# saiprasadbarke/robustmvd

Hardware: AMD Instinct MI355X
Metric: depth-maps/sec at 768x1152x4srcx256planes; warp+aggregate HBM GB/s vs roofline (higher is better)
Workload: dtype f32; 1 GPU; mvsnet (Path B) forward 768x1152, 4 source views, 256 planes, batch 1 per step (BASELINE.json configs[2]); the regulariser's two layers with 32 input channels (conv0, conv4): every fp32 operand as two range-scaled fp16 terms on fp16 MFMA, fp32 accumulation (at least as close to a float64 convolution as the fp32 matrix instruction over 1e-42..1e30: tests/test_hip_f16.py), the other nine layers and ; parallelism=1 independent replica(s), frames round-robin, no collectives

## Files before the change

robustmvd_amd/csrc/conv3d_split.hip:

```cpp
#include "mvd_common.h"
#include "split_operand.h"

#ifndef SPLIT_KO
#define SPLIT_KO 0
#endif
#ifndef SPLIT_DEPTH
#define SPLIT_DEPTH 4
#endif

namespace mvd {

typedef _Float16 h16x8 __attribute__((ext_vector_type(8)));
typedef float sf32x4 __attribute__((ext_vector_type(4)));
typedef unsigned int su32x4 __attribute__((ext_vector_type(4)));
typedef unsigned int su32x2 __attribute__((ext_vector_type(2)));
typedef _Float16 h16x2 __attribute__((ext_vector_type(2)));

constexpr int S_TH = 4, S_TW = 32, S_ROWS = S_TH + 2;
constexpr float S_LO_FACTOR = 2048.0f;
template <int CIN>
struct SplitGeom {
    static constexpr int CH8 = CIN / 8;
    static constexpr int VB = CIN * 2;
    static constexpr int KWG = CIN == 32 ? 3 : 2;
    static constexpr int NT = 9 * KWG;
    static constexpr int COLS = CIN == 32 ? S_TW + 2 : S_TW + 3;
    static constexpr int HALF_BYTES = S_ROWS * COLS * VB;
    static constexpr int PLANE_BYTES = 2 * HALF_BYTES;
    static constexpr int ITEMS = S_ROWS * COLS * CH8;
    static constexpr int NLOAD = (ITEMS + 255) / 256;
    static constexpr int NF = 4 * KWG * 2;
    static_assert(NF - 8 == 4 * NLOAD, "pass B interleaves 8 epilogue groups and 4 staging groups per item");
};

template <int CIN>
__global__ void pack_conv0_split_kernel(const float* __restrict__ w, const float* __restrict__ wscale, _Float16* __restrict__ packed, int ncb) {
    using G = SplitGeom<CIN>;
    const int e = blockIdx.x * 256 + threadIdx.x;
    if (e >= ncb * G::NT * 64 * 8) return;
    const int j = e & 7, lane = (e >> 3) & 63, t = (e >> 9) % G::NT, cb = (e >> 9) / G::NT;
    const int col = lane & 15, k = 8 * (lane >> 4) + j, cout = cb * 8 + (col & 7);
    int tap, cin;
    if constexpr (CIN == 32) { tap = t; cin = k; }
    else { const int kw = 2 * (t % 2) + k / 16; tap = kw < 3 ? (t / 2) * 3 + kw : -1; cin = k % 16; }
    const float v = tap >= 0 ? w[((size_t)cout * CIN + cin) * 27 + tap] / wscale[cout] : 0.0f;
    _Float16 hi, lo;
    split_weight(v, S_LO_FACTOR, hi, lo);
    packed[e] = col < 8 ? hi : lo;
}

struct SplitParams {
    const float* x;
    const char* wpk;
    const float* scale;
    const float* shift;
    const float* absmax;
    float* y;
    float* yamax;
    int B, D, h, w, relu;
    int cout, ncb;
    int tiles_x, tiles_y, dgroups, td, tiles_per_xcd;
};

__device__ __forceinline__ unsigned pack_h2(_Float16 a, _Float16 b) {
    const h16x2 v = {a, b};
    return __builtin_bit_cast(unsigned, v);
}

template <int CIN, bool YAMAX = false>
__global__ void __launch_bounds__(256, 2) conv0_split_kernel(SplitParams p) {
    using G = SplitGeom<CIN>;
    constexpr int S_COLS = G::COLS, S_HALF_BYTES = G::HALF_BYTES, S_PLANE_BYTES = G::PLANE_BYTES, S_ITEMS = G::ITEMS, S_NLOAD = G::NLOAD;
    constexpr int KWG = G::KWG, NT = G::NT;
    extern __shared__ __attribute__((aligned(16))) char ring[];
    const int tid = threadIdx.x, lane = tid & 63, wv = tid >> 6;
    const int D = p.D, h = p.h, w = p.w;

    const int xcd = blockIdx.x & 7;
    int j = blockIdx.x >> 3;
    const int cb = j % p.ncb; j /= p.ncb;
    const int t_in = j % p.tiles_per_xcd; j /= p.tiles_per_xcd;
    const int dg = j % p.dgroups;
    const int b = j / p.dgroups;
    const int tile = xcd * p.tiles_per_xcd + t_in;
    if (tile >= p.tiles_x * p.tiles_y) return;
    const int ty = tile / p.tiles_x, tx = tile - ty * p.tiles_x;
    const int x0 = tx * S_TW, y0 = ty * S_TH;
    const int dz0 = dg * p.td, dz1 = min(dz0 + p.td, D);

    h16x8 wf[NT];
#pragma unroll
    for (int t = 0; t < NT; ++t) wf[t] = *reinterpret_cast<const h16x8*>(p.wpk + (((size_t)cb * NT + t) * 64 + lane) * 16);

    constexpr unsigned OOB = 0x80000000u;
    unsigned gob[S_NLOAD];
    int loff[S_NLOAD];
#pragma unroll
    for (int k = 0; k < S_NLOAD; ++k) {
        const int e = tid + 256 * k;
        const int vox = e / G::CH8, ch = e % G::CH8;
        const int r = vox / S_COLS, c = vox - r * S_COLS;
        const int gy = y0 - 1 + r, gx = x0 - 1 + c;
        const bool in = e < S_ITEMS && c < S_TW + 2 && gy >= 0 && gy < h && gx >= 0 && gx < w;
        gob[k] = in ? (unsigned)(((gy * w + gx) * CIN + ch * 8) * 4) : OOB;
        if constexpr (CIN == 32) loff[k] = e < S_ITEMS ? (vox * 64 + ((ch ^ ((c >> 1) & 3)) * 16)) : -1;
        else loff[k] = e < S_ITEMS ? e * 16 : -1;
    }
    const size_t plane_f = (size_t)h * w * CIN;
    const float* xb = p.x + (size_t)b * D * plane_f;
    su32x4 pre[S_NLOAD][2];
    auto fetch = [&](int d) {
        const bool din = d >= 0 && d < D && d <= dz1;
        const __amdgpu_buffer_rsrc_t rs = __builtin_amdgcn_make_buffer_rsrc(
            const_cast<float*>(xb + (din ? (size_t)d * plane_f : 0)), 0, din ? (int)(plane_f * 4) : 0, 0x00020000);
#pragma unroll
        for (int k = 0; k < S_NLOAD; ++k) {
            pre[k][0] = __builtin_amdgcn_raw_buffer_load_b128(rs, gob[k], 0, 0);
            pre[k][1] = __builtin_amdgcn_raw_buffer_load_b128(rs, gob[k] + 16u, 0, 0);
        }
    };
    char* const dump = ring + 2 * S_PLANE_BYTES + tid * 16;
    float xs, xs_inv;
    split_xscale(p.absmax, xs, xs_inv);
    auto split2 = [xs](float a0, float a1, unsigned& hi, unsigned& lo) { mvd::split2(xs, a0, a1, hi, lo, S_LO_FACTOR); };
    auto stash = [&](int d) {
        char* slot = ring + (d & 1) * S_PLANE_BYTES;
#pragma unroll
        for (int k = 0; k < S_NLOAD; ++k) {
            su32x4 hv, lv;
#pragma unroll
            for (int q = 0; q < 4; ++q) {
                const sf32x4 v = __builtin_bit_cast(sf32x4, pre[k][q >> 1]);
                unsigned hi, lo;
                split2(v[(q & 1) * 2], v[(q & 1) * 2 + 1], hi, lo);
                hv[q] = hi; lv[q] = lo;
            }
            char* dst = loff[k] >= 0 ? slot + loff[k] : dump;
            *reinterpret_cast<su32x4*>(dst) = hv;
            *reinterpret_cast<su32x4*>(loff[k] >= 0 ? dst + S_HALF_BYTES : dst) = lv;
        }
    };

    const int col = lane & 15;
    float esc_ = p.scale[cb * 8 + (col & 7)], esh_ = p.shift[cb * 8 + (col & 7)];
    float eun_ = reinterpret_cast<const float*>(p.wpk + (size_t)p.ncb * NT * 64 * 16)[cb * 8 + (col & 7)] * xs_inv;
    const float floor_ = p.relu ? 0.f : -__builtin_inff();
    const int xh = wv & 1, rp = wv >> 1;

    int fragk[KWG];
#pragma unroll
    for (int kw = 0; kw < KWG; ++kw) {
        if constexpr (CIN == 32) {
            const int c = 16 * xh + (lane & 15) + kw;
            fragk[kw] = (2 * rp * S_COLS + c) * 64 + (((lane >> 4) ^ ((c >> 1) & 3)) * 16);
        } else {
            const int c = 16 * xh + (lane & 15) + 2 * kw;
            fragk[kw] = (2 * rp * S_COLS + c) * 32 + (lane >> 4) * 16;
        }
    }

    sf32x4 acc[3][2][2];
#pragma unroll
    for (int s = 0; s < 3; ++s)
#pragma unroll
        for (int r = 0; r < 2; ++r) { acc[s][r][0] = sf32x4{0, 0, 0, 0}; acc[s][r][1] = sf32x4{0, 0, 0, 0}; }

    unsigned yoff[2];
#pragma unroll
    for (int row = 0; row < 2; ++row) {
        const int oy = y0 + 2 * rp + row;
        yoff[row] = (col < 8 && oy < h) ? (unsigned)((((size_t)oy * w + x0 + 16 * xh + 4 * (lane >> 4)) * p.cout + cb * 8 + col) * 4) : OOB;
    }
    const int oxb = x0 + 16 * xh + 4 * (lane >> 4);
    const size_t yplane_f = (size_t)h * w * p.cout;
    const unsigned vox_b = (unsigned)p.cout * 4u;

    fetch(dz0 - 1);
    asm volatile("" : "+v"(esc_), "+v"(esh_), "+v"(eun_));
    stash(dz0 - 1);
    fetch(dz0);

    [[maybe_unused]] float amax_ = 0.f;
    for (int z = dz0 - 1; z <= dz1; ++z) {
        if (!(SPLIT_KO & 8)) __syncthreads();
        const char* slot = ring + (z & 1) * S_PLANE_BYTES;
        char* wslot = ring + ((z + 1) & 1) * S_PLANE_BYTES;
        const int din = z + 2, dout = z - 1;
        const bool in_ok = din >= 0 && din < D && din <= dz1, out_ok = dout >= dz0 && dout < dz1;
        const __amdgpu_buffer_rsrc_t rs_in = __builtin_amdgcn_make_buffer_rsrc(
            const_cast<float*>(xb + (in_ok ? (size_t)din * plane_f : 0)), 0, in_ok ? (int)(plane_f * 4) : 0, 0x00020000);
        const __amdgpu_buffer_rsrc_t rs_out = __builtin_amdgcn_make_buffer_rsrc(
            p.y + ((size_t)b * D + (out_ok ? dout : 0)) * yplane_f, 0, out_ok ? (int)(yplane_f * 4) : 0, 0x00020000);
        int ox = oxb;
        asm volatile("" : "+v"(ox));

        constexpr int NF = G::NF, NR = 2 * NF, DEPTH = SPLIT_DEPTH;
        h16x8 fr[DEPTH];
        auto rr_of = [](int ro) { return ro == 0 ? 1 : ro == 1 ? 2 : ro == 2 ? 0 : 3; };
        auto frag = [&](int i) {
            const int g = i % NF, term = g & 1, kw = (g >> 1) % KWG, rr = rr_of(g / (2 * KWG));
            if (SPLIT_KO & 32) return wf[i % NT];
            return *reinterpret_cast<const h16x8*>(slot + term * S_HALF_BYTES + fragk[kw] + rr * S_COLS * G::VB);
        };
#pragma unroll
        for (int i = 0; i < DEPTH; ++i) fr[i] = frag(i);
#pragma unroll
        for (int g = 0; g < NF; ++g) {
            const int term = g & 1, kw = (g >> 1) % KWG, rr = rr_of(g / (2 * KWG));
            const h16x8 f = fr[g % DEPTH];
#pragma unroll
            for (int row = 0; row < 2; ++row) {
                const int kh = rr - row;
                if (kh < 0 || kh > 2) continue;
                if (SPLIT_KO & 16) acc[0][row][term][0] += f[0] * wf[(6 + kh) * KWG + kw][0];
                else acc[0][row][term] = __builtin_amdgcn_mfma_f32_16x16x32_f16(f, wf[(6 + kh) * KWG + kw], acc[0][row][term], 0, 0, 0);
            }
            fr[g % DEPTH] = frag(g + DEPTH);
            __builtin_amdgcn_sched_barrier(0);
        }
        float hl = __shfl_down(acc[0][0][0][0], 8, 16);
        unsigned hq0 = 0, lq0 = 0;
#pragma unroll
        for (int g = 0; g < NF; ++g) {
            const int term = g & 1, kw = (g >> 1) % KWG, rr = rr_of(g / (2 * KWG));
            const h16x8 f = fr[(NF + g) % DEPTH];
#pragma unroll
            for (int row = 0; row < 2; ++row) {
                const int kh = rr - row;
                if (kh < 0 || kh > 2) continue;
#pragma unroll
                for (int s = 1; s < 3; ++s)
                    if (SPLIT_KO & 16) acc[s][row][term][0] += f[0] * wf[((2 - s) * 3 + kh) * KWG + kw][0];
                    else acc[s][row][term] = __builtin_amdgcn_mfma_f32_16x16x32_f16(f, wf[((2 - s) * 3 + kh) * KWG + kw], acc[s][row][term], 0, 0, 0);
            }
            if (NF + g + DEPTH < NR) fr[(NF + g) % DEPTH] = frag(NF + g + DEPTH);
            if (g < 8) {
                const int row = g >> 2, i = g & 3;
                const float cur = hl;
                if (g + 1 < 8) hl = __shfl_down(acc[0][(g + 1) >> 2][0][(g + 1) & 3], 8, 16);
                float r = __builtin_fmaf(cur + acc[0][row][1][i], 1.0f / 2048.0f, acc[0][row][0][i]);
                r = fmaxf(__builtin_fmaf(r * eun_, esc_, esh_), floor_);
                if constexpr (YAMAX)
                    if (out_ok && yoff[row] != OOB && ox + i < w) amax_ = fmaxf(amax_, finite_abs_or_zero(r));
                if (!(SPLIT_KO & 2) || r == 12345.678f)
                    __builtin_amdgcn_raw_buffer_store_b32(__float_as_uint(r), rs_out, ox + i < w ? yoff[row] + vox_b * i : OOB, 0, 0);
            } else if (!(SPLIT_KO & 4)) {
                const int k = (g - 8) >> 2, q = (g - 8) & 3;
                const sf32x4 v = __builtin_bit_cast(sf32x4, pre[k][q >> 1]);
                unsigned hq1, lq1;
                split2(v[(q & 1) * 2], v[(q & 1) * 2 + 1], hq1, lq1);
                if (q & 1) {
                    char* dst = (loff[k] >= 0 ? wslot + loff[k] : dump) + 8 * (q >> 1);
                    *reinterpret_cast<su32x2*>(dst) = su32x2{hq0, hq1};
                    *reinterpret_cast<su32x2*>(loff[k] >= 0 ? dst + S_HALF_BYTES : dst) = su32x2{lq0, lq1};
                } else {
                    hq0 = hq1; lq0 = lq1;
                }
                if (q == 3 && !(SPLIT_KO & 1)) {
                    pre[k][0] = __builtin_amdgcn_raw_buffer_load_b128(rs_in, gob[k], 0, 0);
                    pre[k][1] = __builtin_amdgcn_raw_buffer_load_b128(rs_in, gob[k] + 16u, 0, 0);
                }
            }
            __builtin_amdgcn_sched_barrier(0);
        }
#pragma unroll
        for (int r = 0; r < 2; ++r)
#pragma unroll
            for (int t = 0; t < 2; ++t) {
                acc[0][r][t] = acc[1][r][t];
                acc[1][r][t] = acc[2][r][t];
                acc[2][r][t] = sf32x4{0, 0, 0, 0};
            }
    }
    if constexpr (YAMAX) {
        for (int o = 32; o > 0; o >>= 1) amax_ = fmaxf(amax_, __shfl_xor(amax_, o));
        __syncthreads();
        float* wm = reinterpret_cast<float*>(ring);
        if (lane == 0) wm[wv] = amax_;
        __syncthreads();
        if (tid == 0) {
            amax_ = fmaxf(fmaxf(wm[0], wm[1]), fmaxf(wm[2], wm[3]));
            raise_absmax(p.yamax, amax_);
        }
    }
}

}

static bool split_shape_ok(int Cin, int Cout) { return (Cin == 32 || Cin == 16) && Cout >= 8 && Cout <= 64 && Cout % 8 == 0; }
static size_t split_frag_bytes(int Cin, int Cout) { return (size_t)(Cout / 8) * (Cin == 32 ? 27 : 18) * 64 * 16; }

template <int CIN, bool YAMAX>
static int launch_split_v(const mvd::SplitParams& p, long long nblk, hipStream_t st) {
    const size_t lds = 2 * (size_t)mvd::SplitGeom<CIN>::PLANE_BYTES + 256 * 16;
    (void)hipFuncSetAttribute((const void*)mvd::conv0_split_kernel<CIN, YAMAX>, hipFuncAttributeMaxDynamicSharedMemorySize, (int)lds);
    hipLaunchKernelGGL((mvd::conv0_split_kernel<CIN, YAMAX>), dim3((unsigned)nblk), dim3(256), lds, st, p);
    return mvd::launch_status("conv3d_split");
}
template <int CIN>
static int launch_split(const mvd::SplitParams& p, long long nblk, hipStream_t st) {
    return p.yamax ? launch_split_v<CIN, true>(p, nblk, st) : launch_split_v<CIN, false>(p, nblk, st);
}

extern "C" {

size_t mvd_conv3d_split_packed_weight_bytes(int Cin, int Cout) {
    return split_shape_ok(Cin, Cout) ? split_frag_bytes(Cin, Cout) + (size_t)Cout * sizeof(float) : 0;
}

int mvd_pack_conv3d_weights_split(const float* w, int Cin, int Cout, void* packed, mvd_stream_t stream) {
    MVD_REQUIRE(w && packed, "pack_conv3d_weights_split: NULL argument");
    MVD_REQUIRE(split_shape_ok(Cin, Cout), "pack_conv3d_weights_split: 16 or 32 input channels and 8, 16, ... 64 output channels are built (got %d -> %d)", Cin, Cout);
    const int ncb = Cout / 8;
    float* wscale = reinterpret_cast<float*>(static_cast<char*>(packed) + split_frag_bytes(Cin, Cout));
    mvd::split_wscale_launch(w, wscale, Cin, Cout, 27, false, Cout, Cout, (hipStream_t)stream);
    const unsigned nb = (unsigned)((split_frag_bytes(Cin, Cout) / 2 + 255) / 256);
    if (Cin == 32) hipLaunchKernelGGL(mvd::pack_conv0_split_kernel<32>, dim3(nb), dim3(256), 0, (hipStream_t)stream, w, wscale, (_Float16*)packed, ncb);
    else hipLaunchKernelGGL(mvd::pack_conv0_split_kernel<16>, dim3(nb), dim3(256), 0, (hipStream_t)stream, w, wscale, (_Float16*)packed, ncb);
    return mvd::launch_status("pack_conv3d_weights_split");
}

static int conv3d_split_entry(const float* x, const float* x_absmax, const void* packed_w, const float* scale, const float* shift, float* y,
                              float* y_absmax, int B, int D, int h, int w, int Cin, int Cout, int relu, mvd_stream_t stream);

int mvd_conv3d_bn_relu_f32_split(const float* x, const float* x_absmax, const void* packed_w, const float* scale, const float* shift,
                                 float* y, int B, int D, int h, int w, int Cin, int Cout, int relu, mvd_stream_t stream) {
    return conv3d_split_entry(x, x_absmax, packed_w, scale, shift, y, nullptr, B, D, h, w, Cin, Cout, relu, stream);
}

int mvd_conv3d_bn_relu_absmax_f32_split(const float* x, const float* x_absmax, const void* packed_w, const float* scale, const float* shift,
                                        float* y, float* y_absmax, int B, int D, int h, int w, int Cin, int Cout, int relu,
                                        mvd_stream_t stream) {
    MVD_REQUIRE(y_absmax, "conv3d_split_absmax: NULL argument");
    return conv3d_split_entry(x, x_absmax, packed_w, scale, shift, y, y_absmax, B, D, h, w, Cin, Cout, relu, stream);
}

static int conv3d_split_entry(const float* x, const float* x_absmax, const void* packed_w, const float* scale, const float* shift, float* y,
                              float* y_absmax, int B, int D, int h, int w, int Cin, int Cout, int relu, mvd_stream_t stream) {
    MVD_REQUIRE(x && x_absmax && packed_w && scale && shift && y, "conv3d_split: NULL argument");
    MVD_REQUIRE(split_shape_ok(Cin, Cout), "conv3d_split: 16 or 32 input channels and 8, 16, ... 64 output channels are built (got %d -> %d)", Cin, Cout);
    MVD_REQUIRE(B > 0 && D > 0 && h > 0 && w > 0, "conv3d_split: non-positive dimension");
    MVD_REQUIRE((long long)h * w * Cin * 4 < 0x7fffffffLL && (long long)h * w * Cout * 4 < 0x7fffffffLL,
                "conv3d_split: one plane exceeds the 31-bit byte-offset range");
    mvd::SplitParams p{};
    p.x = x; p.absmax = x_absmax; p.wpk = (const char*)packed_w; p.scale = scale; p.shift = shift; p.y = y; p.yamax = y_absmax;
    if (y_absmax && hipMemsetAsync(y_absmax, 0, sizeof(float), (hipStream_t)stream) != hipSuccess) return mvd::launch_status("conv3d_split: memset");
    p.B = B; p.D = D; p.h = h; p.w = w; p.relu = relu;
    p.cout = Cout; p.ncb = Cout / 8;
    p.tiles_x = (w + mvd::S_TW - 1) / mvd::S_TW;
    p.tiles_y = (h + mvd::S_TH - 1) / mvd::S_TH;
    const long long tiles = (long long)p.tiles_x * p.tiles_y;
    p.tiles_per_xcd = (int)((tiles + 7) / 8);
    int td = 32;
    while (td > 8 && tiles * B * p.ncb * ((D + td - 1) / td) < 2048) td /= 2;
    p.td = td;
    p.dgroups = (D + td - 1) / td;
    const long long nblk = 8LL * p.ncb * p.tiles_per_xcd * p.dgroups * B;
    MVD_REQUIRE(nblk <= 0x7fffffffLL, "conv3d_split: %lld workgroups exceed the grid limit", nblk);
    return Cin == 32 ? launch_split<32>(p, nblk, (hipStream_t)stream) : launch_split<16>(p, nblk, (hipStream_t)stream);
}
}
```

Measured before the change: 358.2 depth-maps/sec.

## Share depth-rolling accumulators across split terms and shift results with DPP rotates

The default path (non-SIX) repacks the weights so each fragment packs hi and lo weight terms for two depth taps in its 16 output columns. The depth-sliding accumulator state then shrinks from six per-term accumulators to five (X, Z, LA, Y, LB), with cross-lane DPP row rotates replacing the old shuffle and register shift between depth planes. This is meant to cut the number of MFMAs per plane and drop the shuffle in the epilogue. The change also adds an env-gated persistent-slot scheduler, a configurable staging point and a legacy switch. These add code complexity and make the weight layout depend on how the kernel is built.

```diff
diff --git a/robustmvd_amd/csrc/conv3d_split.hip b/robustmvd_amd/csrc/conv3d_split.hip
--- a/robustmvd_amd/csrc/conv3d_split.hip
+++ b/robustmvd_amd/csrc/conv3d_split.hip
@@ -1,3 +1,6 @@
+#include <algorithm>
+#include <cstdlib>
+
 #include "mvd_common.h"
 #include "split_operand.h"
 
@@ -6,6 +9,9 @@
 #endif
 #ifndef SPLIT_DEPTH
 #define SPLIT_DEPTH 4
+#endif
+#ifndef SPLIT_STAGE_AT
+#define SPLIT_STAGE_AT 8
 #endif
 
 namespace mvd {
@@ -30,23 +36,34 @@
     static constexpr int ITEMS = S_ROWS * COLS * CH8;
     static constexpr int NLOAD = (ITEMS + 255) / 256;
     static constexpr int NF = 4 * KWG * 2;
-    static_assert(NF - 8 == 4 * NLOAD, "pass B interleaves 8 epilogue groups and 4 staging groups per item");
+    static_assert(NF - 8 == 4 * NLOAD, "a pass has room for 8 epilogue groups and 4 staging groups per item");
 };
 
-template <int CIN>
+template <int CIN, bool SIX>
 __global__ void pack_conv0_split_kernel(const float* __restrict__ w, const float* __restrict__ wscale, _Float16* __restrict__ packed, int ncb) {
     using G = SplitGeom<CIN>;
     const int e = blockIdx.x * 256 + threadIdx.x;
     if (e >= ncb * G::NT * 64 * 8) return;
     const int j = e & 7, lane = (e >> 3) & 63, t = (e >> 9) % G::NT, cb = (e >> 9) / G::NT;
     const int col = lane & 15, k = 8 * (lane >> 4) + j, cout = cb * 8 + (col & 7);
+    int kdkh, g;
+    bool lo_term;
+    if constexpr (SIX) {
+        kdkh = t / G::KWG; g = t % G::KWG; lo_term = col >= 8;
+    } else {
+        const int f = t % 3, kh = (t / 3) / G::KWG;
+        g = (t / 3) % G::KWG;
+        const int kd = f == 1 ? 0 : (col < 8 ? 2 : 1);
+        kdkh = kd * 3 + kh;
+        lo_term = f == 2 || (f == 1 && col >= 8);
+    }
     int tap, cin;
-    if constexpr (CIN == 32) { tap = t; cin = k; }
-    else { const int kw = 2 * (t % 2) + k / 16; tap = kw < 3 ? (t / 2) * 3 + kw : -1; cin = k % 16; }
+    if constexpr (CIN == 32) { tap = kdkh * 3 + g; cin = k; }
+    else { const int kw = 2 * g + k / 16; tap = kw < 3 ? kdkh * 3 + kw : -1; cin = k % 16; }
     const float v = tap >= 0 ? w[((size_t)cout * CIN + cin) * 27 + tap] / wscale[cout] : 0.0f;
     _Float16 hi, lo;
     split_weight(v, S_LO_FACTOR, hi, lo);
-    packed[e] = col < 8 ? hi : lo;
+    packed[e] = lo_term ? lo : hi;
 }
 
 struct SplitParams {
@@ -60,6 +77,8 @@
     int B, D, h, w, relu;
     int cout, ncb;
     int tiles_x, tiles_y, dgroups, td, tiles_per_xcd;
+    int slots;
+    long long total;
 };
 
 __device__ __forceinline__ unsigned pack_h2(_Float16 a, _Float16 b) {
@@ -67,7 +86,12 @@
     return __builtin_bit_cast(unsigned, v);
 }
 
-template <int CIN, bool YAMAX = false>
+template <int BANK_MASK>
+__device__ __forceinline__ float ror8(float keep, float src) {
+    return __builtin_bit_cast(float, __builtin_amdgcn_update_dpp(__builtin_bit_cast(int, keep), __builtin_bit_cast(int, src), 0x128, 0xf, BANK_MASK, false));
+}
+
+template <int CIN, bool YAMAX = false, bool SIX = false>
 __global__ void __launch_bounds__(256, 2) conv0_split_kernel(SplitParams p) {
     using G = SplitGeom<CIN>;
     constexpr int S_COLS = G::COLS, S_HALF_BYTES = G::HALF_BYTES, S_PLANE_BYTES = G::PLANE_BYTES, S_ITEMS = G::ITEMS, S_NLOAD = G::NLOAD;
@@ -77,24 +101,83 @@
     const int D = p.D, h = p.h, w = p.w;
 
     const int xcd = blockIdx.x & 7;
-    int j = blockIdx.x >> 3;
-    const int cb = j % p.ncb; j /= p.ncb;
-    const int t_in = j % p.tiles_per_xcd; j /= p.tiles_per_xcd;
-    const int dg = j % p.dgroups;
-    const int b = j / p.dgroups;
-    const int tile = xcd * p.tiles_per_xcd + t_in;
-    if (tile >= p.tiles_x * p.tiles_y) return;
+    long long lin, lin_end;
+    if (p.slots > 0) {
+        const int q = p.slots >> 3, rem = p.slots & 7;
+        const int rank = (xcd < rem ? xcd * (q + 1) : rem * (q + 1) + (xcd - rem) * q) + (int)(blockIdx.x >> 3);
+        lin = p.total * rank / p.slots;
+        lin_end = p.total * (rank + 1) / p.slots;
+    } else {
+        int j = blockIdx.x >> 3;
+        const int cb = j % p.ncb; j /= p.ncb;
+        const int t_in = j % p.tiles_per_xcd; j /= p.tiles_per_xcd;
+        const int dg = j % p.dgroups;
+        const int b = j / p.dgroups;
+        const int tile = xcd * p.tiles_per_xcd + t_in;
+        if (tile >= p.tiles_x * p.tiles_y) return;
+        lin = (((long long)tile * p.B + b) * p.ncb + cb) * D + dg * p.td;
+        lin_end = lin + min(p.td, D - dg * p.td);
+    }
+
+    constexpr unsigned OOB = 0x80000000u;
+    int loff[S_NLOAD];
+#pragma unroll
+    for (int k = 0; k < S_NLOAD; ++k) {
+        const int e = tid + 256 * k;
+        const int vox = e / G::CH8, ch = e % G::CH8;
+        const int c = vox % S_COLS;
+        if constexpr (CIN == 32) loff[k] = e < S_ITEMS ? (vox * 64 + ((ch ^ ((c >> 1) & 3)) * 16)) : -1;
+        else loff[k] = e < S_ITEMS ? e * 16 : -1;
+    }
+    const size_t plane_f = (size_t)h * w * CIN;
+    char* const dump = ring + 2 * S_PLANE_BYTES + tid * 16;
+    float xs, xs_inv;
+    split_xscale(p.absmax, xs, xs_inv);
+    auto split2 = [xs](float a0, float a1, unsigned& hi, unsigned& lo) { mvd::split2(xs, a0, a1, hi, lo, S_LO_FACTOR); };
+    const int col = lane & 15;
+    const float floor_ = p.relu ? 0.f : -__builtin_inff();
+    const int xh = wv & 1, rp = wv >> 1;
+
+    int fragk[KWG];
+#pragma unroll
+    for (int kw = 0; kw < KWG; ++kw) {
+        if constexpr (CIN == 32) {
+            const int c = 16 * xh + (lane & 15) + kw;
+            fragk[kw] = (2 * rp * S_COLS + c) * 64 + (((lane >> 4) ^ ((c >> 1) & 3)) * 16);
+        } else {
+            const int c = 16 * xh + (lane & 15) + 2 * kw;
+            fragk[kw] = (2 * rp * S_COLS + c) * 32 + (lane >> 4) * 16;
+        }
+    }
+    const size_t yplane_f = (size_t)h * w * p.cout;
+    const unsigned vox_b = (unsigned)p.cout * 4u;
+
+    h16x8 wf[NT];
+    float esc_ = 0.f, esh_ = 0.f, eun_ = 0.f;
+    int cb_resident = -1;
+    [[maybe_unused]] float amax_ = 0.f;
+
+  while (lin < lin_end) {
+    const int dz0 = (int)(lin % D);
+    long long sj = lin / D;
+    const int cb = (int)(sj % p.ncb); sj /= p.ncb;
+    const int b = (int)(sj % p.B);
+    const int tile = (int)(sj / p.B);
+    const int dz1 = (int)min((long long)D, dz0 + (lin_end - lin));
+    lin += dz1 - dz0;
     const int ty = tile / p.tiles_x, tx = tile - ty * p.tiles_x;
     const int x0 = tx * S_TW, y0 = ty * S_TH;
-    const int dz0 = dg * p.td, dz1 = min(dz0 + p.td, D);
-
-    h16x8 wf[NT];
-#pragma unroll
-    for (int t = 0; t < NT; ++t) wf[t] = *reinterpret_cast<const h16x8*>(p.wpk + (((size_t)cb * NT + t) * 64 + lane) * 16);
-
-    constexpr unsigned OOB = 0x80000000u;
+
+    if (cb != cb_resident) {
+        cb_resident = cb;
+#pragma unroll
+        for (int t = 0; t < NT; ++t) wf[t] = *reinterpret_cast<const h16x8*>(p.wpk + (((size_t)cb * NT + t) * 64 + lane) * 16);
+        esc_ = p.scale[cb * 8 + (col & 7)];
+        esh_ = p.shift[cb * 8 + (col & 7)];
+        eun_ = reinterpret_cast<const float*>(p.wpk + (size_t)p.ncb * NT * 64 * 16)[cb * 8 + (col & 7)] * xs_inv;
+    }
+
     unsigned gob[S_NLOAD];
-    int loff[S_NLOAD];
 #pragma unroll
     for (int k = 0; k < S_NLOAD; ++k) {
         const int e = tid + 256 * k;
@@ -103,10 +186,7 @@
         const int gy = y0 - 1 + r, gx = x0 - 1 + c;
         const bool in = e < S_ITEMS && c < S_TW + 2 && gy >= 0 && gy < h && gx >= 0 && gx < w;
         gob[k] = in ? (unsigned)(((gy * w + gx) * CIN + ch * 8) * 4) : OOB;
-        if constexpr (CIN == 32) loff[k] = e < S_ITEMS ? (vox * 64 + ((ch ^ ((c >> 1) & 3)) * 16)) : -1;
-        else loff[k] = e < S_ITEMS ? e * 16 : -1;
-    }
-    const size_t plane_f = (size_t)h * w * CIN;
+    }
     const float* xb = p.x + (size_t)b * D * plane_f;
     su32x4 pre[S_NLOAD][2];
     auto fetch = [&](int d) {
@@ -119,10 +199,6 @@
             pre[k][1] = __builtin_amdgcn_raw_buffer_load_b128(rs, gob[k] + 16u, 0, 0);
         }
     };
-    char* const dump = ring + 2 * S_PLANE_BYTES + tid * 16;
-    float xs, xs_inv;
-    split_xscale(p.absmax, xs, xs_inv);
-    auto split2 = [xs](float a0, float a1, unsigned& hi, unsigned& lo) { mvd::split2(xs, a0, a1, hi, lo, S_LO_FACTOR); };
     auto stash = [&](int d) {
         char* slot = ring + (d & 1) * S_PLANE_BYTES;
 #pragma unroll
@@ -141,29 +217,13 @@
         }
     };
 
-    const int col = lane & 15;
-    float esc_ = p.scale[cb * 8 + (col & 7)], esh_ = p.shift[cb * 8 + (col & 7)];
-    float eun_ = reinterpret_cast<const float*>(p.wpk + (size_t)p.ncb * NT * 64 * 16)[cb * 8 + (col & 7)] * xs_inv;
-    const float floor_ = p.relu ? 0.f : -__builtin_inff();
-    const int xh = wv & 1, rp = wv >> 1;
-
-    int fragk[KWG];
-#pragma unroll
-    for (int kw = 0; kw < KWG; ++kw) {
-        if constexpr (CIN == 32) {
-            const int c = 16 * xh + (lane & 15) + kw;
-            fragk[kw] = (2 * rp * S_COLS + c) * 64 + (((lane >> 4) ^ ((c >> 1) & 3)) * 16);
-        } else {
-            const int c = 16 * xh + (lane & 15) + 2 * kw;
-            fragk[kw] = (2 * rp * S_COLS + c) * 32 + (lane >> 4) * 16;
-        }
-    }
-
-    sf32x4 acc[3][2][2];
+    constexpr sf32x4 ZERO4 = {0, 0, 0, 0};
+    [[maybe_unused]] sf32x4 X[2] = {ZERO4, ZERO4}, Z[2] = {ZERO4, ZERO4}, LA[2] = {ZERO4, ZERO4}, Y[2] = {ZERO4, ZERO4}, LB[2] = {ZERO4, ZERO4};
+    [[maybe_unused]] sf32x4 acc[3][2][2];
 #pragma unroll
     for (int s = 0; s < 3; ++s)
 #pragma unroll
-        for (int r = 0; r < 2; ++r) { acc[s][r][0] = sf32x4{0, 0, 0, 0}; acc[s][r][1] = sf32x4{0, 0, 0, 0}; }
+        for (int r = 0; r < 2; ++r) { acc[s][r][0] = ZERO4; acc[s][r][1] = ZERO4; }
 
     unsigned yoff[2];
 #pragma unroll
@@ -172,15 +232,15 @@
         yoff[row] = (col < 8 && oy < h) ? (unsigned)((((size_t)oy * w + x0 + 16 * xh + 4 * (lane >> 4)) * p.cout + cb * 8 + col) * 4) : OOB;
     }
     const int oxb = x0 + 16 * xh + 4 * (lane >> 4);
-    const size_t yplane_f = (size_t)h * w * p.cout;
-    const unsigned vox_b = (unsigned)p.cout * 4u;
 
     fetch(dz0 - 1);
     asm volatile("" : "+v"(esc_), "+v"(esh_), "+v"(eun_));
     stash(dz0 - 1);
     fetch(dz0);
 
-    [[maybe_unused]] float amax_ = 0.f;
+    constexpr int STAGE_AT = SIX || SPLIT_STAGE_AT < 0 ? G::NF + 8 : SPLIT_STAGE_AT;
+    static_assert(STAGE_AT >= 0 && STAGE_AT + 4 * S_NLOAD <= 2 * G::NF && (STAGE_AT >= G::NF + 8 || STAGE_AT + 4 * S_NLOAD <= G::NF),
+                  "the staging groups fit into one step, clear of the epilogue groups");
     for (int z = dz0 - 1; z <= dz1; ++z) {
         if (!(SPLIT_KO & 8)) __syncthreads();
         const char* slot = ring + (z & 1) * S_PLANE_BYTES;
@@ -204,48 +264,26 @@
         };
 #pragma unroll
         for (int i = 0; i < DEPTH; ++i) fr[i] = frag(i);
-#pragma unroll
-        for (int g = 0; g < NF; ++g) {
-            const int term = g & 1, kw = (g >> 1) % KWG, rr = rr_of(g / (2 * KWG));
-            const h16x8 f = fr[g % DEPTH];
-#pragma unroll
-            for (int row = 0; row < 2; ++row) {
-                const int kh = rr - row;
-                if (kh < 0 || kh > 2) continue;
-                if (SPLIT_KO & 16) acc[0][row][term][0] += f[0] * wf[(6 + kh) * KWG + kw][0];
-                else acc[0][row][term] = __builtin_amdgcn_mfma_f32_16x16x32_f16(f, wf[(6 + kh) * KWG + kw], acc[0][row][term], 0, 0, 0);
-            }
-            fr[g % DEPTH] = frag(g + DEPTH);
-            __builtin_amdgcn_sched_barrier(0);
-        }
-        float hl = __shfl_down(acc[0][0][0][0], 8, 16);
+        [[maybe_unused]] float hl = 0.f;
         unsigned hq0 = 0, lq0 = 0;
-#pragma unroll
-        for (int g = 0; g < NF; ++g) {
-            const int term = g & 1, kw = (g >> 1) % KWG, rr = rr_of(g / (2 * KWG));
-            const h16x8 f = fr[(NF + g) % DEPTH];
-#pragma unroll
-            for (int row = 0; row < 2; ++row) {
-                const int kh = rr - row;
-                if (kh < 0 || kh > 2) continue;
-#pragma unroll
-                for (int s = 1; s < 3; ++s)
-                    if (SPLIT_KO & 16) acc[s][row][term][0] += f[0] * wf[((2 - s) * 3 + kh) * KWG + kw][0];
-                    else acc[s][row][term] = __builtin_amdgcn_mfma_f32_16x16x32_f16(f, wf[((2 - s) * 3 + kh) * KWG + kw], acc[s][row][term], 0, 0, 0);
-            }
-            if (NF + g + DEPTH < NR) fr[(NF + g) % DEPTH] = frag(NF + g + DEPTH);
-            if (g < 8) {
-                const int row = g >> 2, i = g & 3;
-                const float cur = hl;
-                if (g + 1 < 8) hl = __shfl_down(acc[0][(g + 1) >> 2][0][(g + 1) & 3], 8, 16);
-                float r = __builtin_fmaf(cur + acc[0][row][1][i], 1.0f / 2048.0f, acc[0][row][0][i]);
+        auto ride = [&](int si) {
+            if (si >= NF && si < NF + 8) {
+                const int g = si - NF, row = g >> 2, i = g & 3;
+                float r;
+                if constexpr (SIX) {
+                    const float cur = hl;
+                    if (g + 1 < 8) hl = __shfl_down(acc[0][(g + 1) >> 2][0][(g + 1) & 3], 8, 16);
+                    r = __builtin_fmaf(cur + acc[0][row][1][i], 1.0f / 2048.0f, acc[0][row][0][i]);
+                } else {
+                    r = __builtin_fmaf(Z[row][i] + LA[row][i], 1.0f / 2048.0f, X[row][i]);
+                }
                 r = fmaxf(__builtin_fmaf(r * eun_, esc_, esh_), floor_);
                 if constexpr (YAMAX)
                     if (out_ok && yoff[row] != OOB && ox + i < w) amax_ = fmaxf(amax_, finite_abs_or_zero(r));
                 if (!(SPLIT_KO & 2) || r == 12345.678f)
                     __builtin_amdgcn_raw_buffer_store_b32(__float_as_uint(r), rs_out, ox + i < w ? yoff[row] + vox_b * i : OOB, 0, 0);
-            } else if (!(SPLIT_KO & 4)) {
-                const int k = (g - 8) >> 2, q = (g - 8) & 3;
+            } else if (si >= STAGE_AT && si < STAGE_AT + 4 * S_NLOAD && !(SPLIT_KO & 4)) {
+                const int k = (si - STAGE_AT) >> 2, q = (si - STAGE_AT) & 3;
                 const sf32x4 v = __builtin_bit_cast(sf32x4, pre[k][q >> 1]);
                 unsigned hq1, lq1;
                 split2(v[(q & 1) * 2], v[(q & 1) * 2 + 1], hq1, lq1);
@@ -261,17 +299,80 @@
                     pre[k][1] = __builtin_amdgcn_raw_buffer_load_b128(rs_in, gob[k] + 16u, 0, 0);
                 }
             }
+        };
+        auto mma = [](const h16x8& a, const h16x8& b, sf32x4& c) {
+            if (SPLIT_KO & 16) c[0] += a[0] * b[0];
+            else c = __builtin_amdgcn_mfma_f32_16x16x32_f16(a, b, c, 0, 0, 0);
+        };
+#pragma unroll
+        for (int g = 0; g < NF; ++g) {
+            const int term = g & 1, kw = (g >> 1) % KWG, rr = rr_of(g / (2 * KWG));
+            const h16x8 f = fr[g % DEPTH];
+#pragma unroll
+            for (int row = 0; row < 2; ++row) {
+                const int kh = rr - row;
+                if (kh < 0 || kh > 2) continue;
+                if constexpr (SIX) {
+                    mma(f, wf[(6 + kh) * KWG + kw], acc[0][row][term]);
+                } else if (term == 0) {
+                    mma(f, wf[(kh * KWG + kw) * 3 + 0], X[row]);
+                    mma(f, wf[(kh * KWG + kw) * 3 + 2], Z[row]);
+                } else {
+                    mma(f, wf[(kh * KWG + kw) * 3 + 0], LA[row]);
+                }
+            }
+            fr[g % DEPTH] = frag(g + DEPTH);
+            ride(g);
             __builtin_amdgcn_sched_barrier(0);
         }
-#pragma unroll
-        for (int r = 0; r < 2; ++r)
-#pragma unroll
-            for (int t = 0; t < 2; ++t) {
-                acc[0][r][t] = acc[1][r][t];
-                acc[1][r][t] = acc[2][r][t];
-                acc[2][r][t] = sf32x4{0, 0, 0, 0};
+        if constexpr (SIX) hl = __shfl_down(acc[0][0][0][0], 8, 16);
+#pragma unroll
+        for (int g = 0; g < NF; ++g) {
+            const int term = g & 1, kw = (g >> 1) % KWG, rr = rr_of(g / (2 * KWG));
+            const h16x8 f = fr[(NF + g) % DEPTH];
+#pragma unroll
+            for (int row = 0; row < 2; ++row) {
+                const int kh = rr - row;
+                if (kh < 0 || kh > 2) continue;
+                if constexpr (SIX) {
+#pragma unroll
+                    for (int s = 1; s < 3; ++s) {
+                        if ((SPLIT_KO & 64) && s == 1 && term == 1) continue;
+                        mma(f, wf[((2 - s) * 3 + kh) * KWG + kw], acc[s][row][term]);
+                    }
+                } else {
+                    mma(f, wf[(kh * KWG + kw) * 3 + 1], term == 0 ? Y[row] : LB[row]);
+                }
             }
-    }
+            if (NF + g + DEPTH < NR) fr[(NF + g) % DEPTH] = frag(NF + g + DEPTH);
+            ride(NF + g);
+            __builtin_amdgcn_sched_barrier(0);
+        }
+        if constexpr (SIX) {
+#pragma unroll
+            for (int r = 0; r < 2; ++r)
+#pragma unroll
+                for (int t = 0; t < 2; ++t) {
+                    acc[0][r][t] = acc[1][r][t];
+                    acc[1][r][t] = acc[2][r][t];
+                    acc[2][r][t] = ZERO4;
+                }
+        } else {
+            constexpr int LOW = 0x3, HIGH = 0xc;
+#pragma unroll
+            for (int r = 0; r < 2; ++r)
+#pragma unroll
+                for (int i = 0; i < 4; ++i) {
+                    X[r][i] = ror8<HIGH>(ror8<LOW>(X[r][i], X[r][i]), Y[r][i]);
+                    Z[r][i] = ror8<LOW>(Y[r][i], Z[r][i]);
+                    LA[r][i] = ror8<HIGH>(ror8<LOW>(LA[r][i], LA[r][i]), LB[r][i]);
+                    Y[r][i] = 0.f;
+                    LB[r][i] = 0.f;
+                }
+        }
+    }
+    if (lin < lin_end) __syncthreads();
+  }
     if constexpr (YAMAX) {
         for (int o = 32; o > 0; o >>= 1) amax_ = fmaxf(amax_, __shfl_xor(amax_, o));
         __syncthreads();
@@ -290,12 +391,21 @@
 static bool split_shape_ok(int Cin, int Cout) { return (Cin == 32 || Cin == 16) && Cout >= 8 && Cout <= 64 && Cout % 8 == 0; }
 static size_t split_frag_bytes(int Cin, int Cout) { return (size_t)(Cout / 8) * (Cin == 32 ? 27 : 18) * 64 * 16; }
 
+static bool split_six() { return mvd::exp_env("MVD_CONV0_LEGACY") != nullptr; }
+
+template <int CIN, bool YAMAX, bool SIX>
+static int launch_split_k(const mvd::SplitParams& p, long long nblk, hipStream_t st) {
+    const size_t lds = 2 * (size_t)mvd::SplitGeom<CIN>::PLANE_BYTES + 256 * 16;
+    (void)hipFuncSetAttribute((const void*)mvd::conv0_split_kernel<CIN, YAMAX, SIX>, hipFuncAttributeMaxDynamicSharedMemorySize, (int)lds);
+    hipLaunchKernelGGL((mvd::conv0_split_kernel<CIN, YAMAX, SIX>), dim3((unsigned)nblk), dim3(256), lds, st, p);
+    return mvd::launch_status("conv3d_split");
+}
 template <int CIN, bool YAMAX>
 static int launch_split_v(const mvd::SplitParams& p, long long nblk, hipStream_t st) {
-    const size_t lds = 2 * (size_t)mvd::SplitGeom<CIN>::PLANE_BYTES + 256 * 16;
-    (void)hipFuncSetAttribute((const void*)mvd::conv0_split_kernel<CIN, YAMAX>, hipFuncAttributeMaxDynamicSharedMemorySize, (int)lds);
-    hipLaunchKernelGGL((mvd::conv0_split_kernel<CIN, YAMAX>), dim3((unsigned)nblk), dim3(256), lds, st, p);
-    return mvd::launch_status("conv3d_split");
+#ifdef MVD_EXPERIMENTS
+    if (split_six()) return launch_split_k<CIN, YAMAX, true>(p, nblk, st);
+#endif
+    return launch_split_k<CIN, YAMAX, false>(p, nblk, st);
 }
 template <int CIN>
 static int launch_split(const mvd::SplitParams& p, long long nblk, hipStream_t st) {
@@ -314,9 +424,17 @@
     const int ncb = Cout / 8;
     float* wscale = reinterpret_cast<float*>(static_cast<char*>(packed) + split_frag_bytes(Cin, Cout));
     mvd::split_wscale_launch(w, wscale, Cin, Cout, 27, false, Cout, Cout, (hipStream_t)stream);
-    const unsigned nb = (unsigned)((split_frag_bytes(Cin, Cout) / 2 + 255) / 256);
-    if (Cin == 32) hipLaunchKernelGGL(mvd::pack_conv0_split_kernel<32>, dim3(nb), dim3(256), 0, (hipStream_t)stream, w, wscale, (_Float16*)packed, ncb);
-    else hipLaunchKernelGGL(mvd::pack_conv0_split_kernel<16>, dim3(nb), dim3(256), 0, (hipStream_t)stream, w, wscale, (_Float16*)packed, ncb);
+    const dim3 nb((unsigned)((split_frag_bytes(Cin, Cout) / 2 + 255) / 256));
+    _Float16* out = (_Float16*)packed;
+#ifdef MVD_EXPERIMENTS
+    if (split_six()) {
+        if (Cin == 32) hipLaunchKernelGGL((mvd::pack_conv0_split_kernel<32, true>), nb, dim3(256), 0, (hipStream_t)stream, w, wscale, out, ncb);
+        else hipLaunchKernelGGL((mvd::pack_conv0_split_kernel<16, true>), nb, dim3(256), 0, (hipStream_t)stream, w, wscale, out, ncb);
+        return mvd::launch_status("pack_conv3d_weights_split");
+    }
+#endif
+    if (Cin == 32) hipLaunchKernelGGL((mvd::pack_conv0_split_kernel<32, false>), nb, dim3(256), 0, (hipStream_t)stream, w, wscale, out, ncb);
+    else hipLaunchKernelGGL((mvd::pack_conv0_split_kernel<16, false>), nb, dim3(256), 0, (hipStream_t)stream, w, wscale, out, ncb);
     return mvd::launch_status("pack_conv3d_weights_split");
 }
 
@@ -351,10 +469,21 @@
     p.tiles_y = (h + mvd::S_TH - 1) / mvd::S_TH;
     const long long tiles = (long long)p.tiles_x * p.tiles_y;
     p.tiles_per_xcd = (int)((tiles + 7) / 8);
+    p.total = tiles * B * p.ncb * D;
+    MVD_REQUIRE(p.total < (1LL << 44), "conv3d_split: %lld planes of tiles exceed the supported range", p.total);
     int td = 32;
     while (td > 8 && tiles * B * p.ncb * ((D + td - 1) / td) < 2048) td /= 2;
+    if (const char* e = mvd::exp_env("MVD_CONV0_TD")) {
+        if (atoi(e) > 0) td = atoi(e);
+    }
     p.td = td;
     p.dgroups = (D + td - 1) / td;
+    int slots = 0;
+    if (const char* e = mvd::exp_env("MVD_CONV0_SLOTS")) slots = atoi(e);
+    if (slots > 0) {
+        p.slots = (int)std::min<long long>(slots, p.total);
+        return Cin == 32 ? launch_split<32>(p, p.slots, (hipStream_t)stream) : launch_split<16>(p, p.slots, (hipStream_t)stream);
+    }
     const long long nblk = 8LL * p.ncb * p.tiles_per_xcd * p.dgroups * B;
     MVD_REQUIRE(nblk <= 0x7fffffffLL, "conv3d_split: %lld workgroups exceed the grid limit", nblk);
     return Cin == 32 ? launch_split<32>(p, nblk, (hipStream_t)stream) : launch_split<16>(p, nblk, (hipStream_t)stream);
```

Result: faster. 363.6 depth-maps/sec, median of 6 (+1.5%).
